# Lzcstan/DrugLAMP

Measured on AMD Instinct MI355X. Metric: drug-protein pairs/sec training step, higher is better.
Workload: dtype bf16; 1 GPU; DrugLAMP training step (cls step, epoch 1; fwd+bwd+grad all-reduce+AdamW), BindingDB-shaped synthetic pairs (512 drug nodes/tokens, 2304 protein tokens = 256 sites, pre-extracted 384-d/640-d LLM embeddings), global batch 256 = 256 per GPU x 1; per_gpu_batch=256, global_batch=256, parallelism=dp1, step_kind=cls, epoch=1, hip_graph=False, protein_seq_len=2304, distinct_batches=8, first_touch_steps=8, padding_rows=computed once, protein_cnn_rows=distinct rows, streams=independent branches on side HIP streams

## Files before the change

### druglamp_amd/_lib.py

```python
from __future__ import annotations

import ctypes as C
import os

import torch

_HERE = os.path.dirname(os.path.abspath(__file__))
_variant = os.environ.get("DL_USE_STUDY_LIB", "")
if _variant and not _variant.endswith(".so"):
    raise RuntimeError("DL_USE_STUDY_LIB=%s: the -DDL_STUDY build (libdruglamp_hip_study.so) was removed; commit 97fb613 is the last "
                       "that builds it (python -m druglamp_amd.build --study).  Only a variant library name (libdruglamp_hip_<variant>.so) "
                       "is accepted." % _variant)
LIB_PATH = os.path.join(_HERE, "lib", _variant or "libdruglamp_hip.so")

DL_F32, DL_BF16 = 0, 1

c_i64, c_i32, c_f32, c_u64, c_vp, c_sz = C.c_int64, C.c_int32, C.c_float, C.c_uint64, C.c_void_p, C.c_size_t


class ReduceItem(C.Structure):
    _fields_ = [
        ("kind", c_i32), ("out_dtype", c_i32),
        ("src", c_vp), ("out", c_vp),
        ("mn", c_i64), ("ldc", c_i64),
# ... 209 lines not shown
    "dl_pgca_pairs_ragged_profile": (c_i32, [C.POINTER(PgcaPairsRaggedProfileArgs), c_vp]),
    "dl_token_gate_fwd": (c_i32, [c_vp, c_vp, c_vp, c_vp, c_i64, c_i64, c_i64, c_i32, c_i32, c_i32, c_vp]),
    "dl_token_gate_bwd": (c_i32, [c_vp, c_vp, c_vp, c_vp, c_vp, c_i64, c_i64, c_i64, c_i32, c_i32, c_i32, c_vp]),
    "dl_gate_dpre": (c_i32, [c_vp, c_vp, c_vp, c_vp, c_i64, c_i64, c_i32, c_i32, c_vp]),
    "dl_add_rowmod_dropout": (c_i32, [c_vp, c_vp, c_vp, c_i64, c_i64, c_i64, c_f32, c_u64, c_vp, c_i32, c_vp]),
    "dl_dropout_apply": (c_i32, [c_vp, c_vp, c_i64, c_i64, c_i64, c_i64, c_f32, c_u64, c_vp, c_i32, c_vp]),
    "dl_fill_pool": (c_i32, [c_vp, c_vp, c_vp, c_i64, c_i64, c_i64, c_i32, c_i32, c_i32, c_vp]),
    "dl_cnn_sitepool_fwd": (c_i32, [c_vp, c_vp, c_i64, c_i64, c_i64, c_i32, c_i32, c_i32, c_vp]),
    "dl_cnn_sitepool_bwd": (c_i32, [c_vp, c_vp, c_i64, c_i64, c_i64, c_i32, c_i32, c_i32, c_vp]),
    "dl_bn_stats_finalize": (c_i32, [c_vp, c_i64, c_i64, c_i64, c_i64, c_i64, c_vp, c_i32, c_i64, c_f32, c_f32, c_vp, c_vp, c_vp, c_vp, c_vp, c_vp, c_vp, c_sz, c_vp]),
    "dl_bn_finalize": (c_i32, [c_vp, c_i64, c_f32, c_f32, c_vp, c_vp, c_vp, c_vp, c_vp, c_i64, c_vp]),
    "dl_interleave_streams": (c_i32, [c_vp, c_vp, c_i64, c_i64, c_i32, c_i32, c_vp]),
    "dl_norm_adjacency": (c_i32, [c_vp, c_vp, c_i64, c_i32, c_i32, c_vp]),
    "dl_graph_aggregate": (c_i32, [c_vp, c_vp, c_vp, c_i64, c_i32, c_i32, c_i32, c_i32, c_i32, c_vp]),
    "dl_concat2": (c_i32, [c_vp, c_vp, c_vp, c_i64, c_i64, c_i64, c_i32, c_vp]),
    "dl_gather_pad": (c_i32, [c_vp, c_vp, c_vp, c_vp, c_i64, c_i64, c_i64, c_i32, c_i32, c_vp]),
    "dl_embed_pad": (c_i32, [c_vp, c_vp, c_vp, c_vp, c_i64, c_i64, c_i32, c_i32, c_i32, c_i32, c_vp]),
    "dl_weight_prep": (c_i32, [c_vp, c_vp, c_i32, c_i32, c_vp]),
    "dl_gelu_bwd": (c_i32, [c_vp, c_vp, c_vp, c_i64, c_i32, c_vp]),
    "dl_cast": (c_i32, [c_vp, c_i32, c_vp, c_i32, c_i64, c_vp]),
    "dl_rowmod_sum": (c_i32, [c_vp, c_vp, c_i64, c_i64, c_i64, c_i32, c_i32, c_vp]),
    "dl_cos_rowloss_fwd": (c_i32, [c_vp, c_vp, c_vp, c_vp, c_i64, c_i64, c_vp]),
    "dl_cos_rowloss_bwd": (c_i32, [c_vp, c_vp, c_f32, c_vp, c_i64, c_i64, c_vp]),
    "dl_ntxent_fwd_ex": (c_i32, [C.POINTER(NtxentArgs), c_vp, c_vp, c_vp, c_vp]),
    "dl_ntxent_bwd_ex": (c_i32, [C.POINTER(NtxentArgs), c_f32, c_vp, c_vp, c_vp]),
    "dl_ntxent_workspace_bytes": (c_sz, [c_i64, c_i64]),
    "dl_ntxent_fwd": (c_i32, [c_vp, c_vp, c_i64, c_i64, c_f32, c_vp, c_vp, c_vp, c_sz, c_vp]),
    "dl_ntxent_bwd": (c_i32, [c_vp, c_vp, c_i64, c_i64, c_f32, c_vp, c_f32, c_vp, c_vp, c_vp]),
    "dl_triplet_sigcos_buffer_floats": (c_sz, [c_i64, c_i64]),
    "dl_triplet_sigcos_fwd": (c_i32, [c_vp, c_vp, c_vp, c_i64, c_i64, c_i64, c_f32, c_vp, c_vp, c_vp, c_vp]),
    "dl_triplet_sigcos_bwd": (c_i32, [c_vp, c_vp, c_vp, c_vp, c_i64, c_i64, c_i64, c_f32, c_vp, c_f32, c_vp, c_vp, c_vp]),
    "dl_adamw_step": (c_i32, [c_vp, c_vp, c_vp, c_vp, c_i64, c_f32, c_f32, c_f32, c_f32, c_f32, c_i64, c_f32, c_vp,
                              c_i32, c_vp]),
    "dl_bn_stats_rw": (c_i32, [c_vp, c_i64, c_i64, c_vp, c_i32, c_vp, c_vp, c_sz, c_vp]),
    "dl_bn_apply_fwd_rw": (c_i32, [c_vp, c_vp, c_vp, c_vp, c_vp, c_vp, c_i64, c_i64, c_vp, c_i32, c_vp]),
    "dl_bn_bwd_reduce_rw": (c_i32, [c_vp, c_vp, c_vp, c_vp, c_i64, c_i64, c_vp, c_i32, c_vp, c_vp, c_sz, c_vp]),
    "dl_bn_bwd_apply_rw": (c_i32, [c_vp, c_vp, c_vp, c_vp, c_vp, c_vp, c_f32, c_i32, c_vp, c_i64, c_i64, c_vp, c_i32, c_vp]),
    "dl_bn_eval_bwd": (c_i32, [c_vp, c_vp, c_vp, c_vp, c_vp, c_vp, c_i32, c_i32, c_vp, c_vp, c_i64, c_i64, c_i64, c_i64, c_i64, c_vp, c_i32,
                               c_vp, c_sz, c_vp]),
    "dl_cnn_sitepool_rows_fwd": (c_i32, [c_vp, c_vp, c_vp, c_i64, c_i64, c_i64, c_i32, c_i32, c_vp]),
    "dl_cnn_sitepool_rows_bwd": (c_i32, [c_vp, c_vp, c_vp, c_vp, c_i64, c_i64, c_i64, c_i64, c_i32, c_i32, c_vp]),
    "dl_embed_rows": (c_i32, [c_vp, c_vp, c_vp, c_vp, c_vp, c_i64, c_i32, c_i32, c_vp, c_i64, c_i64, c_vp, c_i32, c_vp]),
    "dl_rows_gather": (c_i32, [c_vp, c_vp, c_vp, c_i64, c_i64, c_vp]),
    "dl_rows_sum_strided": (c_i32, [c_vp, c_vp, c_vp, c_i64, c_i64, c_i32, c_vp]),
    "dl_rows_equal_check": (c_i32, [c_vp, c_i64, c_i64, c_i64, c_i64, C.c_uint32, c_vp, c_vp]),
    "dl_ce_rows_workspace_bytes": (c_sz, [c_i64]),
    "dl_ce_rows_fwd": (c_i32, [c_vp, c_i64, c_vp, c_i64, c_i32, c_i64, c_i32, c_vp, c_vp, c_vp, c_sz, c_vp]),
    "dl_ce_rows_bwd": (c_i32, [c_vp, c_i64, c_vp, c_i64, c_i32, c_i64, c_i32, c_vp, c_vp, c_vp, c_vp, c_i64, c_i32, c_vp]),
    "dl_protein_plan_build": (c_i32, [c_vp, c_i64, c_i64, c_i64, c_vp, c_vp, c_vp, c_vp, c_vp, c_vp, c_vp]),
    "dl_prof_enable": (c_i32, [c_i32, c_i32]),
    "dl_prof_collect": (c_i32, [c_i32, C.POINTER(c_i64), C.POINTER(C.c_double), C.POINTER(C.c_double),
                                C.POINTER(C.c_double)]),
    "dl_prof_totals": (c_i32, [c_i32, C.POINTER(c_i64), C.POINTER(C.c_double), C.POINTER(C.c_double)]),
    "dl_prof_collect_tag": (c_i32, [c_i32, c_i32, C.POINTER(c_i64), C.POINTER(C.c_double), C.POINTER(C.c_double), C.POINTER(C.c_double),
                                    C.POINTER(c_i64), C.POINTER(C.c_double), C.POINTER(C.c_double)]),
}

_lib = None

AUDIT = os.environ.get("DL_GRAPH_PTR_AUDIT") == "1"
_audit_log = None


def audit_begin() -> None:
    global _audit_log
    _audit_log = []
# ... 80 lines not shown
```

### druglamp_amd/build.py

```python
from __future__ import annotations

import os
import subprocess
import sys
from concurrent.futures import ThreadPoolExecutor

HERE = os.path.dirname(os.path.abspath(__file__))
CSRC = os.path.join(HERE, "csrc")
LIBDIR = os.path.join(HERE, "lib")
OBJDIR = os.path.join(LIBDIR, "obj")
LIB = os.path.join(LIBDIR, "libdruglamp_hip.so")
ARCH = "gfx950"
HIPCC = os.environ.get("HIPCC", "/opt/rocm/bin/hipcc")
FLAGS = ["--offload-arch=" + ARCH, "-O3", "-std=c++17", "-fPIC", "-Wno-unused-result"] + os.environ.get("DL_EXTRA_HIPCC_FLAGS", "").split()


def _sources():
    return sorted(f for f in os.listdir(CSRC) if f.endswith(".hip"))


def _headers():
    hs = [os.path.join(CSRC, f) for f in os.listdir(CSRC) if f.endswith(".cuh")]
    hs.append(os.path.join(os.path.dirname(HERE), "include", "druglamp_hip.h"))
    return hs


def csrc_hash() -> str:
    import hashlib
    h = hashlib.sha1()
    files = [os.path.join(CSRC, f) for f in sorted(os.listdir(CSRC)) if f.endswith((".hip", ".cuh"))]
    files.append(os.path.join(os.path.dirname(HERE), "include", "druglamp_hip.h"))
    for f in files:
        h.update(os.path.basename(f).encode() + b"\0")
        with open(f, "rb") as fh:
            h.update(fh.read())
    return h.hexdigest()


def _stale(out, deps):
    if not os.path.exists(out):
        return True
    t = os.path.getmtime(out)
    return any(os.path.getmtime(d) > t for d in deps)


FILE_FLAGS = {"norm.hip": ["-fno-slp-vectorize"], "elementwise.hip": ["-fno-slp-vectorize"], "bn_eval.hip": ["-fno-slp-vectorize"]}


def _compile(src, force, objdir=OBJDIR, extra=()):
    obj = os.path.join(objdir, src[:-4] + ".o")
    path = os.path.join(CSRC, src)
    if force or _stale(obj, [path] + _headers() + [os.path.abspath(__file__)]):
        keep = os.environ.get("DL_BUILD_NOSLP_FILES")
        ff = FILE_FLAGS.get(src, []) if (keep is None or src in keep.split(",")) else []
        if src in os.environ.get("DL_BUILD_NOSLP_EXTRA", "").split(","):
            ff = ff + ["-fno-slp-vectorize"]
        cmd = [HIPCC] + FLAGS + ff + list(extra) + ["-c", path, "-o", obj]
        r = subprocess.run(cmd, capture_output=True, text=True)
        if r.returncode != 0:
            raise RuntimeError("hipcc failed for %s:\n%s\n%s" % (src, r.stdout, r.stderr))
    return obj


def build(force: bool = False, verbose: bool = True, variant: str = "", defines=()) -> str:
    objdir = OBJDIR + ("_" + variant if variant else "")
    lib = LIB.replace(".so", "_%s.so" % variant) if variant else LIB
    extra = tuple(defines)
    os.makedirs(objdir, exist_ok=True)
    srcs = _sources()
    with ThreadPoolExecutor(max_workers=min(6, len(srcs))) as ex:
        objs = list(ex.map(lambda s: _compile(s, force, objdir, extra), srcs))
    return _link(lib, objs, force, verbose)


def _link(LIB, objs, force, verbose):
    if force or _stale(LIB, objs):
        cmd = [HIPCC, "--offload-arch=" + ARCH, "-shared", "-fPIC", "-o", LIB] + objs
        r = subprocess.run(cmd, capture_output=True, text=True)
        if r.returncode != 0:
# ... 18 lines not shown
```

### druglamp_amd/functional.py

```python
from __future__ import annotations

import functools
import contextlib
import os
import math
import weakref
from typing import List, Optional, Sequence

import torch

from . import ops

_param_epoch = 0
def _maybe_deferring():
    return contextlib.nullcontext() if os.environ.get("DL_DEFER_REDUCTIONS", "1") == "0" else ops.deferred_reductions()


def _deferring(fn):
    if os.environ.get("DL_DEFER_REDUCTIONS", "1") == "0":
        return fn

    @functools.wraps(fn)
    def wrapped(*a, **k):
        with ops.deferred_reductions():
# ... 1196 lines not shown
            ticks, _tick_list = _tick_list, None
            if ticks and exc[0] is None:
                cnt = {}
                for t in ticks:
                    e = cnt.setdefault(id(t), [t, 0])
                    e[1] += 1
                with torch.no_grad():
                    for k in sorted({c for _, c in cnt.values()}):
                        torch._foreach_add_([t for t, c in cnt.values() if c == k], k)
        return False


def bn_tick(counter: torch.Tensor) -> None:
    if _tick_list is not None:
        _tick_list.append(counter)
    else:
        with torch.no_grad():
            counter += 1


def batch_norm_rows(bn: torch.nn.BatchNorm1d, x2d: torch.Tensor, relu: bool = False) -> torch.Tensor:
    C = x2d.shape[1]
    if bn.training and x2d.shape[0] <= 1:
        raise ValueError("Expected more than 1 value per channel when training, got input size {}".format(x2d.size()))
    w = bn.weight if bn.weight is not None else torch.ones(C, device=x2d.device)
    b = bn.bias if bn.bias is not None else torch.zeros(C, device=x2d.device)
    y, mean, var = BatchNormRowsFn.apply(x2d, w, b, bn.running_mean, bn.running_var, bn.training, bn.eps,
                                         bn.momentum if bn.training else None, relu)
    if bn.training:
        bn_tick(bn.num_batches_tracked)
    return y


def run_mlp(seq, x: torch.Tensor, tail=None) -> torch.Tensor:
    import torch.nn as nn
    layers = list(seq)
    i = 0
    while i < len(layers):
        layer = layers[i]
        if isinstance(layer, nn.Linear):
            if x.shape[-1] < layer.in_features:
                raise ValueError("run_mlp: input narrower than the layer")
            x = dense(x, layer.weight, layer.bias)
        elif isinstance(layer, nn.BatchNorm1d):
            if x.shape[-1] != layer.num_features:
                x = x[:, :layer.num_features].contiguous()
            fuse = i + 1 < len(layers) and isinstance(layers[i + 1], nn.ReLU)
            if tail is not None and layer.training:
                x = batch_norm_rows_weighted_tail(layer, x, *tail, relu=fuse)
            else:
                x = batch_norm_rows(layer, x, relu=fuse)
            i += 1 if fuse else 0
        elif isinstance(layer, nn.ReLU):
            x = torch.relu(x)
        else:
            raise NotImplementedError("run_mlp: %s" % type(layer).__name__)
        i += 1
    return x
```

### druglamp_amd/model/basic_model.py

```python
from __future__ import annotations

import contextlib

import os

import torch
import torch.nn as nn
import torch.nn.functional as F

from .. import functional as Fn
from .. import ops
from .. import screening
from ..configs import get_model_defaults
from .cross_modality import CrossModality
from .PGCA import GuidedCrossAttention
from .PMMA import MultiHeadLinearAttention, PairedMultimodelAttention
from .self_supervised_learning import SSL

from .._lib import FLAG_DRUG_TOKEN_PAD as _FLAG_TOK, FLAG_GCN_NODE_PAD as _FLAG_GCN

_TAIL_ROWS = 8

CONFIGS = {"LAMP": get_model_defaults}

# ... 165 lines not shown
        if bn_training:
            for bn in (self.bn1, self.bn2, self.bn3):
                Fn.bn_tick(bn.num_batches_tracked)
        if fused_pool:
            return z
        z = z.transpose(1, 2).contiguous().view(B, L, C)
        if site_pool:
            z = z.view(B, int(site_pool), L // int(site_pool), C).mean(dim=1)
        return z


class FeedForwardLayer(nn.Module):
    def __init__(self, d_in, d_h):
        super().__init__()
        self.lin1 = nn.Linear(d_in, d_h)
        self.lin2 = nn.Linear(d_h, d_in)
        self.act = nn.GELU()
        self.norm = nn.LayerNorm(d_h)

    def forward(self, x):
        return self.lin2(self.norm(self.act(self.lin1(x))))


class MLP(nn.Module):
    def __init__(self, in_dim, hidden_dim, out_dim, binary=1):
        super().__init__()
        self.fc1 = nn.Linear(in_dim, hidden_dim)
        self.bn1 = nn.BatchNorm1d(hidden_dim)
        self.fc2 = nn.Linear(hidden_dim, hidden_dim)
        self.bn2 = nn.BatchNorm1d(hidden_dim)
        self.fc3 = nn.Linear(hidden_dim, out_dim)
        self.bn3 = nn.BatchNorm1d(out_dim)
        self.fc4 = nn.Linear(out_dim, binary)

    compute_dtype = torch.float32

    def forward(self, x):
        x = Fn.cast(x, self.compute_dtype)
        for fc, bn in ((self.fc1, self.bn1), (self.fc2, self.bn2), (self.fc3, self.bn3)):
            x = Fn.batch_norm_rows(bn, Fn.dense(x, fc.weight, fc.bias, act=True))
        return Fn.dense(x, self.fc4.weight, self.fc4.bias)[:, :self.fc4.out_features]


class DrugLAMPBase(nn.Module):
    llm_branch = True

    def __init__(self, n_drug_feature, n_prot_feature, n_hidden=128, **cfg):
        super().__init__()
        self.site_len = cfg["PROTEIN"]["SITE_LEN"]
        self.seq_len_q = cfg["PROTEIN"]["SEQ_LEN"]
        dec = cfg["DECODER"]
        self.compact_padding = os.environ.get("DL_PAD_COMPACT", "1") != "0"
        self.check_padding = os.environ.get("DL_PAD_CHECK", "0") == "1"
        self.guard_padding = os.environ.get("DL_PAD_GUARD", "1") != "0"
        self.compact_cnn = os.environ.get("DL_CNN_COMPACT", "1") != "0"
        self.compact_keys = os.environ.get("DL_KEY_COMPACT", "1") != "0"
        self.branch_streams = os.environ.get("DL_BRANCH_STREAMS", "1") != "0"
        self._streams = None
        self.drug_extractor = MolecularGCN(in_feats=cfg["DRUG"]["NODE_IN_FEATS"], dim_embedding=n_hidden,
                                           padding=cfg["DRUG"]["PADDING"], hidden_feats=[n_hidden] * 3)
        self.protein_extractor = ProteinCNN(n_hidden, [n_hidden] * 3, cfg["PROTEIN"]["KERNEL_SIZE"],
                                            cfg["PROTEIN"]["PADDING"])
        self.ssl_model = SSL(prot_extractor=self.protein_extractor, n_prot_feature=n_prot_feature,
                             drug_ssl_type=str(cfg["RS"].get("DRUG_SSL_TYPE", "simsiam")), n_hidden=n_hidden,
                             global_batch=bool(cfg["RS"].get("GLOBAL_BATCH", False)))
        self.cm_model = CrossModality(use_cm=True, hidden_size=n_hidden, max_margin=cfg["RS"]["MAX_MARGIN"],
                                      n_re=cfg["RS"]["RESET_EPOCH"], global_batch=bool(cfg["RS"].get("GLOBAL_BATCH", False)))
        if self.seq_len_q % self.site_len:
            raise ValueError("PROTEIN.SEQ_LEN (%d) must be a multiple of PROTEIN.SITE_LEN (%d)" % (self.seq_len_q, self.site_len))
        model_cfg = CONFIGS["LAMP"](n_hidden, feat_len=self.seq_len_q // self.site_len)

        self.lin_d1 = nn.Linear(n_drug_feature + 1, 2 * n_hidden)
# ... 297 lines not shown
```

### druglamp_amd/ops.py

```python
from __future__ import annotations

import contextlib
import ctypes as C
import math
import os
from typing import Optional

import torch

from . import _lib
from ._lib import (DL_BF16, DL_F32, AttnBwdArgs, AttnFwdArgs, AttnProbsArgs, GemmArgs, PgcaPairsArgs, PgcaPairsProbsArgs, PgcaPairsProfileArgs,
                   PgcaPairsRaggedArgs, PgcaPairsRaggedProbsArgs, PgcaPairsRaggedProfileArgs, check)

_DT = {torch.float32: DL_F32, torch.bfloat16: DL_BF16}


def _dt(t: torch.Tensor) -> int:
    try:
        return _DT[t.dtype]
    except KeyError:
        raise TypeError("druglamp_amd: unsupported dtype %s (float32 / bfloat16 only)" % t.dtype)


_raw_stream = getattr(torch._C, "_cuda_getCurrentRawStream", None)
# ... 871 lines not shown
    lse = torch.empty(N, dtype=torch.float32, device=logits2d.device)
    out2 = torch.empty(2, dtype=torch.float32, device=logits2d.device)
    ws = _ws2.get(L.dl_ce_rows_workspace_bytes(N), logits2d.device)
    check(L.dl_ce_rows_fwd(logits2d.data_ptr(), ld, labels.data_ptr(), N, C, int(ignore_index), _dt(logits2d), lse.data_ptr(),
                           out2.data_ptr(), ws.data_ptr(), ws.numel(), _stream()), "dl_ce_rows_fwd")
    return out2, lse


def ce_rows_bwd(logits2d, labels, C: int, ignore_index: int, lse, out2, grad_out):
    N, Cp = logits2d.shape
    d = torch.empty((N, Cp), dtype=logits2d.dtype, device=logits2d.device)
    check(_lib.lib().dl_ce_rows_bwd(logits2d.data_ptr(), logits2d.stride(0), labels.data_ptr(), N, C, int(ignore_index), _dt(logits2d),
                                    lse.data_ptr(), out2.data_ptr(), grad_out.data_ptr(), d.data_ptr(), Cp, Cp, _stream()), "dl_ce_rows_bwd")
    return d


def gate_dpre(dl2d, w2, pre2d):
    _need_gpu(dl2d, w2, pre2d)
    M, H = dl2d.shape
    dd = pre2d.shape[1]
    out = torch.empty_like(pre2d)
    check(_lib.lib().dl_gate_dpre(dl2d.data_ptr(), w2.data_ptr(), pre2d.data_ptr(), out.data_ptr(), M, dd, H, _dt(pre2d), _stream()),
          "dl_gate_dpre")
    return out


def gelu_bwd(dy2d, pre2d):
    dx = torch.empty_like(dy2d)
    check(_lib.lib().dl_gelu_bwd(dy2d.data_ptr(), pre2d.data_ptr(), dx.data_ptr(), dy2d.numel(), _dt(dy2d), _stream()),
          "dl_gelu_bwd")
    return dx


def fill_pool(x: torch.Tensor, site_len: int, out_dtype: torch.dtype):
    _need_gpu(x)
    x = x.contiguous()
    B, S, F = x.shape
    Fp = (F + 1 + 7) // 8 * 8
    fill = torch.empty((B, S), dtype=x.dtype, device=x.device)
    pooled = torch.empty((B, S // site_len, Fp), dtype=out_dtype, device=x.device)
    check(_lib.lib().dl_fill_pool(x.data_ptr(), fill.data_ptr(), pooled.data_ptr(), B, S, F, site_len, _dt(x),
                                  _DT[out_dtype], _stream()), "dl_fill_pool")
    return fill, pooled


_weight_prep_launches = 0


def weight_prep_launches() -> int:
    return _weight_prep_launches


def weight_prep(items_dev: torch.Tensor, block_map_dev: torch.Tensor, n_blocks: int, out_dtype: torch.dtype) -> None:
    global _weight_prep_launches
    _need_gpu(items_dev, block_map_dev)
    _weight_prep_launches += 1
    check(_lib.lib().dl_weight_prep(items_dev.data_ptr(), block_map_dev.data_ptr(), int(n_blocks), _DT[out_dtype],
                                    _stream()), "dl_weight_prep")


def cnn_sitepool_fwd(z: torch.Tensor, L: int, halo: int, site_len: int) -> torch.Tensor:
    _need_gpu(z)
    B, LP, C = z.shape
    out = torch.empty((B, L // site_len, C), dtype=z.dtype, device=z.device)
    check(_lib.lib().dl_cnn_sitepool_fwd(z.data_ptr(), out.data_ptr(), B, L, C, halo, site_len, _dt(z), _stream()),
          "dl_cnn_sitepool_fwd")
# ... 208 lines not shown
```

### include/druglamp_hip.h

```cpp
#ifndef DRUGLAMP_HIP_H
#define DRUGLAMP_HIP_H

#include <stddef.h>
#include <stdint.h>

#ifdef __cplusplus
extern "C" {
#endif

typedef enum { DL_OK = 0, DL_ERR_ARG = -1, DL_ERR_SHAPE = -2, DL_ERR_ALIGN = -3,
               DL_ERR_WORKSPACE = -4, DL_ERR_LAUNCH = -5, DL_ERR_UNSUPPORTED = -6 } dl_status;

typedef enum { DL_F32 = 0, DL_BF16 = 1 } dl_dtype;

typedef void* dl_stream;

const char* dl_last_error(void);
int dl_version(void);

typedef struct dl_reduce_item {
  int32_t kind;
  int32_t out_dtype;
  const float* src;
  void* out;
// ... 50 lines not shown
int dl_bn_stats(const void* y, int64_t R, int64_t C, int64_t win, int64_t halo, int64_t valid,
                int32_t dtype, float* sums, void* workspace, size_t workspace_bytes, dl_stream s);
int dl_bn_finalize(const float* sums, int64_t n, float eps, float momentum, float* mean, float* var, float* rstd,
                   float* running_mean, float* running_var, int64_t C, dl_stream s);
int dl_bn_apply_fwd(const void* y, void* z, const float* mean, const float* rstd, const float* gamma,
                    const float* beta, int64_t R, int64_t C, int64_t win, int64_t halo, int64_t valid,
                    int32_t dtype, dl_stream s);
int dl_bn_bwd_reduce(const void* dz, const void* y, const float* mean, const float* rstd, int64_t R,
                     int64_t C, int64_t win, int64_t halo, int64_t valid, int32_t dtype, float* sums,
                     void* workspace, size_t workspace_bytes, dl_stream s);
int dl_bn_bwd_apply(const void* dz, const void* y, const float* mean, const float* rstd,
                    const float* gamma, const float* sums, float inv_n, int32_t relu_mask, void* dy,
                    int64_t R, int64_t C, int64_t win, int64_t halo, int64_t valid, int32_t dtype,
                    dl_stream s);
int dl_bn_stats_rw(const void* y, int64_t R, int64_t C, const float* row_w, int32_t dtype, float* sums, void* workspace,
                   size_t workspace_bytes, dl_stream s);
int dl_bn_stats_finalize(const void* y, int64_t R, int64_t C, int64_t win, int64_t halo, int64_t valid, const float* row_w,
                         int32_t dtype, int64_t n, float eps, float momentum, float* sums, float* mean, float* var, float* rstd,
                         float* running_mean, float* running_var, void* workspace, size_t workspace_bytes, dl_stream s);
int dl_bn_apply_fwd_rw(const void* y, void* z, const float* mean, const float* rstd, const float* gamma, const float* beta,
                       int64_t R, int64_t C, const float* row_w, int32_t dtype, dl_stream s);
int dl_bn_bwd_reduce_rw(const void* dz, const void* y, const float* mean, const float* rstd, int64_t R, int64_t C,
                        const float* row_w, int32_t dtype, float* sums, void* workspace, size_t workspace_bytes, dl_stream s);
int dl_bn_bwd_apply_rw(const void* dz, const void* y, const float* mean, const float* rstd, const float* gamma,
                       const float* sums, float inv_n, int32_t relu_mask, void* dy, int64_t R, int64_t C, const float* row_w,
                       int32_t dtype, dl_stream s);
int dl_bn_tail_fix(void* dy, const void* y, const float* mean, const float* rstd, const float* gamma, const float* sums,
                   float inv_n, int32_t w, int64_t R, int64_t C, int64_t win, int64_t lead, int32_t dtype, dl_stream s);
int dl_bn_apply_relu_fwd(const void* y, void* z, const float* mean, const float* rstd, const float* gamma, const float* beta,
                         int64_t R, int64_t C, int32_t dtype, dl_stream s);
int dl_bn_relu_bwd(const void* dz, const void* y, const float* mean, const float* rstd, const float* gamma, const float* beta,
                   float inv_n, void* dy, float* sums, int64_t R, int64_t C, int32_t dtype, void* workspace, size_t workspace_bytes,
                   dl_stream s);
int dl_bn_eval_bwd(const void* dz, const void* y, const float* mean, const float* rstd, const float* gamma, const float* beta,
                   int32_t relu_in, int32_t relu_out, void* dy, float* sums, int64_t R, int64_t C, int64_t win, int64_t halo,
                   int64_t valid, const float* row_w, int32_t dtype, void* workspace, size_t workspace_bytes, dl_stream s);

int dl_layernorm_fwd(const void* x, int64_t ldx, const float* gamma, const float* beta, void* y,
                     int64_t ldy, float* mean, float* rstd, int64_t M, int64_t D, float eps,
                     int32_t dtype, dl_stream s);
size_t dl_layernorm_bwd_workspace_bytes(int64_t M, int64_t D);
int dl_layernorm_bwd(const void* dy, int64_t lddy, int64_t dy_share, const void* x, int64_t ldx, const float* mean,
                     const float* rstd, const float* gamma, const void* dres, int64_t lddres,
                     void* dx, int64_t lddx, float* dgamma, float* dbeta, int32_t accumulate,
                     int64_t M, int64_t D, int32_t dtype, void* workspace, size_t workspace_bytes,
                     dl_reduce_item* deferred, dl_stream s);

typedef struct {
  const void* Q; const void* K; const void* V; void* O; float* LSE; float* raw_logits;
  int64_t q_ps, q_hs, q_rs, k_ps, k_hs, k_rs, v_ps, v_hs, v_rs, o_ps, o_hs, o_rs, o_ss;
  int32_t n_problems, n_heads, n_segments, partner_shift, Lq, Lk, head_dim, dtype;
  float scale;
  int32_t algo;
  int32_t key_tail_rows;
  float key_tail_weight;
} dl_attn_fwd_args;
enum { DL_ATTN_ALGO_AUTO = 0, DL_ATTN_ALGO_STREAM = 1, DL_ATTN_ALGO_TWO_PASS = 2, DL_ATTN_ALGO_ONE_PASS = 3 };
int dl_attn_fwd(const dl_attn_fwd_args* a, dl_stream s);

typedef struct {
  const void* Q; const void* K; const void* V; const void* O; const void* dO;
  const float* LSE; float* Delta;
  void* dQ; void* dK; void* dV;
  int64_t q_ps, q_hs, q_rs, k_ps, k_hs, k_rs, v_ps, v_hs, v_rs, o_ps, o_hs, o_rs, o_ss;
  int64_t do_ps, do_hs, do_rs, do_ss, dq_ps, dq_hs, dq_rs, dk_ps, dk_hs, dk_rs, dv_ps, dv_hs, dv_rs;
  int32_t n_problems, n_heads, n_segments, partner_shift, Lq, Lk, head_dim, dtype;
// ... 209 lines not shown
```

Measured before the change: 21250 pairs/s.

## Fuse MLP head Linear+GELU+BatchNorm into single forward and backward kernels

Adds HIP kernels that run each decoder-head layer (linear, bias, GELU, training-mode BatchNorm with running-stat update) in one workgroup per 32 output columns, holding every batch row so the column statistics are reduced on chip. The backward kernel fuses the BN and GELU gradients with the dbias/dgamma/dbeta reductions and computes dW slices over a K-split grid; dx still uses a separate GEMM. The goal is to cut kernel launches and intermediate round trips through memory for these small MLP layers. It is enabled by default for bf16 batches of up to 256 rows and adds narrow shape constraints; grids are small (N/32 workgroups), so occupancy may be low.

Measured after the change: 21370 pairs/s, median of 4. Within noise of the previous version (+0.6%).

```diff
diff --git a/druglamp_amd/_lib.py b/druglamp_amd/_lib.py
--- a/druglamp_amd/_lib.py
+++ b/druglamp_amd/_lib.py
@@ -265,6 +265,8 @@
     "dl_triplet_sigcos_bwd": (c_i32, [c_vp, c_vp, c_vp, c_vp, c_i64, c_i64, c_i64, c_f32, c_vp, c_f32, c_vp, c_vp, c_vp]),
     "dl_adamw_step": (c_i32, [c_vp, c_vp, c_vp, c_vp, c_i64, c_f32, c_f32, c_f32, c_f32, c_f32, c_i64, c_f32, c_vp,
                               c_i32, c_vp]),
+    "dl_head_layer_fwd": (c_i32, [c_vp, c_vp, c_vp, c_vp, c_vp, c_vp, c_vp, c_vp, c_vp, c_vp, c_vp, c_i64, c_i64, c_i64, c_f32, c_f32, c_i32, c_vp]),
+    "dl_head_layer_bwd": (c_i32, [c_vp, c_vp, c_vp, c_vp, c_vp, c_vp, c_vp, c_vp, c_vp, c_vp, c_vp, c_i64, c_i64, c_i64, c_i32, c_vp]),
     "dl_bn_stats_rw": (c_i32, [c_vp, c_i64, c_i64, c_vp, c_i32, c_vp, c_vp, c_sz, c_vp]),
     "dl_bn_apply_fwd_rw": (c_i32, [c_vp, c_vp, c_vp, c_vp, c_vp, c_vp, c_i64, c_i64, c_vp, c_i32, c_vp]),
     "dl_bn_bwd_reduce_rw": (c_i32, [c_vp, c_vp, c_vp, c_vp, c_i64, c_i64, c_vp, c_i32, c_vp, c_vp, c_sz, c_vp]),
diff --git a/druglamp_amd/build.py b/druglamp_amd/build.py
--- a/druglamp_amd/build.py
+++ b/druglamp_amd/build.py
@@ -44,7 +44,8 @@
     return any(os.path.getmtime(d) > t for d in deps)
 
 
-FILE_FLAGS = {"norm.hip": ["-fno-slp-vectorize"], "elementwise.hip": ["-fno-slp-vectorize"], "bn_eval.hip": ["-fno-slp-vectorize"]}
+FILE_FLAGS = {"norm.hip": ["-fno-slp-vectorize"], "elementwise.hip": ["-fno-slp-vectorize"], "bn_eval.hip": ["-fno-slp-vectorize"],
+              "head.hip": ["-fno-slp-vectorize"]}
 
 
 def _compile(src, force, objdir=OBJDIR, extra=()):
diff --git a/druglamp_amd/csrc/head.hip b/druglamp_amd/csrc/head.hip
--- /dev/null
+++ b/druglamp_amd/csrc/head.hip
@@ -0,0 +1,350 @@
+#include "tiles.cuh"
+
+namespace {
+using namespace dltile;
+
+constexpr int HL_ROWS = 256;
+constexpr int HL_COLS = 32;
+constexpr int HL_KC = 64;
+constexpr int HL_KSPAN = 128;
+constexpr int HL_PF = 4;
+using XT = ATile<bf16_t, HL_KC>;
+
+template <int NR> struct ChunkStager {
+  static_assert((NR * XT::CPR) % 256 == 0, "every thread stages the same number of 16-byte pieces");
+  static constexpr int NCH = NR * XT::CPR / 256;
+  u32x4 r[NCH];
+  uint32_t ok;
+  __device__ __forceinline__ void load(const bf16_t* __restrict__ base, int64_t ld, int row0, int row_limit, int col0, int col_limit) {
+    ok = 0u;
+#pragma unroll
+    for (int i = 0; i < NCH; ++i) {
+      const int c = threadIdx.x + i * 256;
+      const int row = row0 + c / XT::CPR, col = col0 + (c % XT::CPR) * 8;
+      if (row < row_limit && col < col_limit) ok |= 1u << i;
+      r[i] = *reinterpret_cast<const u32x4*>(base + (int64_t)min(row, row_limit - 1) * ld + min(col, col_limit - 8));
+    }
+  }
+  __device__ __forceinline__ void store(char* lds) const {
+#pragma unroll
+    for (int i = 0; i < NCH; ++i) {
+      const int c = threadIdx.x + i * 256;
+      const int row = c / XT::CPR, ch = c % XT::CPR;
+      lds_write16(lds, row * XT::RB + ((ch ^ XT::swz(row)) << 4), ((ok >> i) & 1u) ? r[i] : u32x4{0u, 0u, 0u, 0u});
+    }
+  }
+};
+
+__device__ __forceinline__ f32x4 unpack4(u32x2 w) { return f32x4{bf16lo(w[0]), bf16hi(w[0]), bf16lo(w[1]), bf16hi(w[1])}; }
+__device__ __forceinline__ u32x2 pack4(f32x4 v) { return u32x2{pack_bf16x2(v[0], v[1]), pack_bf16x2(v[2], v[3])}; }
+
+template <int ROUNDS>
+__global__ __launch_bounds__(256) void head_layer_fwd_kernel(const bf16_t* __restrict__ x, const bf16_t* __restrict__ w,
+                                                             const float* __restrict__ bias, const float* __restrict__ gamma,
+                                                             const float* __restrict__ beta, bf16_t* __restrict__ z, bf16_t* __restrict__ y,
+                                                             float* __restrict__ mean, float* __restrict__ rstd, float* __restrict__ rmean,
+                                                             float* __restrict__ rvar, int M, int N, int K, float eps, float momentum,
+                                                             float unbias) {
+  __shared__ __attribute__((aligned(16))) char Xs[HL_ROWS * XT::RB];
+  __shared__ __attribute__((aligned(16))) char Ws[HL_COLS * XT::RB];
+  __shared__ float red[4][HL_COLS];
+  __shared__ __attribute__((aligned(16))) float col_mean[HL_COLS];
+  __shared__ __attribute__((aligned(16))) float col_rstd[HL_COLS];
+  const int tid = threadIdx.x, lane = tid & 63, wave = tid >> 6, il = lane & 15, g = lane >> 4;
+  const int n0 = blockIdx.x * HL_COLS;
+  const int wrow = wave * 64;
+  int nrt = (M - wrow + 15) / 16;
+  nrt = nrt < 0 ? 0 : (nrt > 4 ? 4 : nrt);
+
+  f32x4 acc[2][4];
+#pragma unroll
+  for (int ct = 0; ct < 2; ++ct)
+#pragma unroll
+    for (int rt = 0; rt < 4; ++rt) acc[ct][rt] = f32x4{0.f, 0.f, 0.f, 0.f};
+
+  ChunkStager<HL_ROWS> sx[HL_PF];
+  ChunkStager<HL_COLS> sw[HL_PF];
+#pragma unroll
+  for (int s = 0; s < HL_PF; ++s) {
+    sx[s].load(x, K, 0, M, s * HL_KC, K);
+    sw[s].load(w, K, n0, N, s * HL_KC, K);
+  }
+#pragma unroll
+  for (int r = 0; r < ROUNDS; ++r) {
+#pragma unroll
+    for (int s = 0; s < HL_PF; ++s) {
+      const int k0 = (r * HL_PF + s) * HL_KC;
+      __syncthreads();
+      sx[s].store(Xs);
+      sw[s].store(Ws);
+      __syncthreads();
+      if (r + 1 < ROUNDS) {
+        sx[s].load(x, K, 0, M, k0 + HL_PF * HL_KC, K);
+        sw[s].load(w, K, n0, N, k0 + HL_PF * HL_KC, K);
+      }
+      if (k0 < K) {
+#pragma unroll
+        for (int kf = 0; kf < HL_KC / 32; ++kf) {
+          const u32x4 wa0 = frag_kc<bf16_t, HL_KC>(Ws, 0, kf, il, g), wa1 = frag_kc<bf16_t, HL_KC>(Ws, 16, kf, il, g);
+#pragma unroll
+          for (int rt = 0; rt < 4; ++rt) {
+            if (rt < nrt) {
+              const u32x4 xb = frag_kc<bf16_t, HL_KC>(Xs, wrow + rt * 16, kf, il, g);
+              acc[0][rt] = Mma<bf16_t>::mma(wa0, xb, acc[0][rt]);
+              acc[1][rt] = Mma<bf16_t>::mma(wa1, xb, acc[1][rt]);
+            }
+          }
+        }
+      }
+    }
+  }
+
+  int col[2];
+  bool colok[2];
+  f32x4 b4[2];
+#pragma unroll
+  for (int ct = 0; ct < 2; ++ct) {
+    col[ct] = n0 + ct * 16 + 4 * g;
+    colok[ct] = col[ct] < N;
+    b4[ct] = colok[ct] ? *reinterpret_cast<const f32x4*>(bias + col[ct]) : f32x4{0.f, 0.f, 0.f, 0.f};
+  }
+  f32x4 s[2] = {f32x4{0.f, 0.f, 0.f, 0.f}, f32x4{0.f, 0.f, 0.f, 0.f}};
+#pragma unroll
+  for (int ct = 0; ct < 2; ++ct)
+#pragma unroll
+    for (int rt = 0; rt < 4; ++rt) {
+      const int row = wrow + rt * 16 + il;
+      const bool ok = row < M;
+      const u32x2 zb = pack4(acc[ct][rt] + b4[ct]);
+      if (ok && colok[ct]) *reinterpret_cast<u32x2*>(z + (int64_t)row * N + col[ct]) = zb;
+      const f32x4 a = gelu4<bf16_t>(unpack4(zb));
+      acc[ct][rt] = a;
+      if (ok) s[ct] += a;
+    }
+#pragma unroll
+  for (int ct = 0; ct < 2; ++ct)
+#pragma unroll
+    for (int r = 0; r < 4; ++r) {
+      const float t = row16_sum(s[ct][r]);
+      if (il == 0) red[wave][ct * 16 + 4 * g + r] = t;
+    }
+  __syncthreads();
+  const float inv_m = 1.f / (float)M;
+  if (tid < HL_COLS) col_mean[tid] = (((red[0][tid] + red[1][tid]) + red[2][tid]) + red[3][tid]) * inv_m;
+  __syncthreads();
+  f32x4 mu[2];
+#pragma unroll
+  for (int ct = 0; ct < 2; ++ct) {
+    mu[ct] = *reinterpret_cast<const f32x4*>(&col_mean[ct * 16 + 4 * g]);
+    s[ct] = f32x4{0.f, 0.f, 0.f, 0.f};
+#pragma unroll
+    for (int rt = 0; rt < 4; ++rt) {
+      const f32x4 d = acc[ct][rt] - mu[ct];
+      acc[ct][rt] = d;
+      if (wrow + rt * 16 + il < M) s[ct] += d * d;
+    }
+  }
+#pragma unroll
+  for (int ct = 0; ct < 2; ++ct)
+#pragma unroll
+    for (int r = 0; r < 4; ++r) {
+      const float t = row16_sum(s[ct][r]);
+      if (il == 0) red[wave][ct * 16 + 4 * g + r] = t;
+    }
+  __syncthreads();
+  if (tid < HL_COLS) {
+    const float var = (((red[0][tid] + red[1][tid]) + red[2][tid]) + red[3][tid]) * inv_m;
+    const float rs = rsqrtf(var + eps);
+    col_rstd[tid] = rs;
+    const int c = n0 + tid;
+    if (c < N) {
+      const float m = col_mean[tid];
+      mean[c] = m;
+      rstd[c] = rs;
+      if (rmean) rmean[c] = (1.f - momentum) * rmean[c] + momentum * m;
+      if (rvar) rvar[c] = (1.f - momentum) * rvar[c] + momentum * (var * unbias);
+    }
+  }
+  __syncthreads();
+#pragma unroll
+  for (int ct = 0; ct < 2; ++ct) {
+    if (!colok[ct]) continue;
+    const f32x4 rs = *reinterpret_cast<const f32x4*>(&col_rstd[ct * 16 + 4 * g]);
+    const f32x4 ga = *reinterpret_cast<const f32x4*>(gamma + col[ct]), be = *reinterpret_cast<const f32x4*>(beta + col[ct]);
+#pragma unroll
+    for (int rt = 0; rt < 4; ++rt) {
+      const int row = wrow + rt * 16 + il;
+      if (row < M) *reinterpret_cast<u32x2*>(y + (int64_t)row * N + col[ct]) = pack4(acc[ct][rt] * rs * ga + be);
+    }
+  }
+}
+
+struct DzTile {
+  static constexpr int RB = HL_COLS * 2;
+  __device__ static __forceinline__ int off(int row, int col) {
+    const int b = col * 2;
+    return row * RB + ((((b >> 4) ^ ((row >> 2) & 3))) << 4) + (b & 15);
+  }
+};
+__device__ __forceinline__ u32x4 dz_frag_tr(const char* lds, int rbase, int colbase, int il, int g) {
+  const int r0 = rbase + 4 * g + (il >> 2);
+  const int col = colbase + (il & 3) * 4;
+  const u32x2 a = lds_read_tr16(lds, DzTile::off(r0, col));
+  const u32x2 b = lds_read_tr16(lds, DzTile::off(r0 + 16, col));
+  return u32x4{a[0], a[1], b[0], b[1]};
+}
+
+__device__ __forceinline__ void colsum32(float (*red)[HL_COLS], float* out) {
+  __syncthreads();
+  if (threadIdx.x < HL_COLS) {
+    float t = 0.f;
+#pragma unroll
+    for (int k = 0; k < 32; ++k) t += red[k][threadIdx.x];
+    out[threadIdx.x] = t;
+  }
+  __syncthreads();
+}
+
+__global__ __launch_bounds__(256) void head_layer_bwd_kernel(const bf16_t* __restrict__ dy, const bf16_t* __restrict__ z,
+                                                             const float* __restrict__ mean, const float* __restrict__ rstd,
+                                                             const float* __restrict__ gamma, const bf16_t* __restrict__ xin,
+                                                             bf16_t* __restrict__ dz, float* __restrict__ dW, float* __restrict__ dbias,
+                                                             float* __restrict__ dgamma, float* __restrict__ dbeta, int M, int N, int K) {
+  __shared__ __attribute__((aligned(16))) char Xs[HL_ROWS * XT::RB];
+  __shared__ __attribute__((aligned(16))) char Ds[HL_ROWS * DzTile::RB];
+  __shared__ float red[32][HL_COLS];
+  __shared__ __attribute__((aligned(16))) float sum0[HL_COLS];
+  __shared__ __attribute__((aligned(16))) float sum1[HL_COLS];
+  const int tid = threadIdx.x, lane = tid & 63, wave = tid >> 6, il = lane & 15, g = lane >> 4;
+  const int n0 = blockIdx.x * HL_COLS;
+  const int kbeg = blockIdx.y * HL_KSPAN;
+  const int kend = min(K, kbeg + HL_KSPAN);
+  const bool first = blockIdx.y == 0;
+
+  static_assert(HL_KSPAN == 2 * HL_KC, "the two stagers below hold the workgroup's whole x_in span");
+  ChunkStager<HL_ROWS> sx[2];
+  sx[0].load(xin, K, 0, M, kbeg, K);
+  sx[1].load(xin, K, 0, M, kbeg + HL_KC, K);
+
+  const int cl = (tid & 7) * 4, rsub = tid >> 3;
+  const int cq = n0 + cl;
+  const bool colok = cq < N;
+  f32x4 mu = {0.f, 0.f, 0.f, 0.f}, rs = mu, ga = mu;
+  if (colok) {
+    mu = *reinterpret_cast<const f32x4*>(mean + cq);
+    rs = *reinterpret_cast<const f32x4*>(rstd + cq);
+    ga = *reinterpret_cast<const f32x4*>(gamma + cq);
+  }
+  f32x4 d[8], zr[8], xh[8];
+  f32x4 s0 = {0.f, 0.f, 0.f, 0.f}, s1 = s0;
+#pragma unroll
+  for (int j = 0; j < 8; ++j) {
+    const int row = rsub + 32 * j;
+    d[j] = f32x4{0.f, 0.f, 0.f, 0.f};
+    zr[j] = d[j];
+    if (colok && row < M) {
+      d[j] = unpack4(*reinterpret_cast<const u32x2*>(dy + (int64_t)row * N + cq));
+      zr[j] = unpack4(*reinterpret_cast<const u32x2*>(z + (int64_t)row * N + cq));
+    }
+    xh[j] = (gelu4<bf16_t>(zr[j]) - mu) * rs;
+    if (row < M) { s0 += d[j]; s1 += d[j] * xh[j]; }
+  }
+#pragma unroll
+  for (int e = 0; e < 4; ++e) red[rsub][cl + e] = s0[e];
+  colsum32(red, sum0);
+#pragma unroll
+  for (int e = 0; e < 4; ++e) red[rsub][cl + e] = s1[e];
+  colsum32(red, sum1);
+  const float inv_m = 1.f / (float)M;
+  const f32x4 m0 = *reinterpret_cast<const f32x4*>(&sum0[cl]) * inv_m, m1 = *reinterpret_cast<const f32x4*>(&sum1[cl]) * inv_m;
+  const f32x4 gr = ga * rs;
+  f32x4 s2 = {0.f, 0.f, 0.f, 0.f};
+#pragma unroll
+  for (int j = 0; j < 8; ++j) {
+    const int row = rsub + 32 * j;
+    f32x4 v = {0.f, 0.f, 0.f, 0.f};
+    if (colok && row < M) {
+      const f32x4 da = gr * (d[j] - m0 - xh[j] * m1);
+      v = da * gelu_grad4<bf16_t>(zr[j]);
+      s2 += v;
+    }
+    const u32x2 vb = pack4(v);
+    *reinterpret_cast<u32x2*>(Ds + DzTile::off(row, cl)) = vb;
+    if (first && colok && row < M) *reinterpret_cast<u32x2*>(dz + (int64_t)row * N + cq) = vb;
+  }
+  if (first && tid < HL_COLS && n0 + tid < N) { dbeta[n0 + tid] = sum0[tid]; dgamma[n0 + tid] = sum1[tid]; }
+#pragma unroll
+  for (int e = 0; e < 4; ++e) red[rsub][cl + e] = s2[e];
+  colsum32(red, sum0);
+  if (first && tid < HL_COLS && n0 + tid < N) dbias[n0 + tid] = sum0[tid];
+
+  const int nfr = (M + 31) / 32;
+#pragma unroll
+  for (int s = 0; s < 2; ++s) {
+    const int k0 = kbeg + s * HL_KC;
+    if (k0 >= kend) break;
+    __syncthreads();
+    sx[s].store(Xs);
+    __syncthreads();
+    f32x4 acc[2] = {f32x4{0.f, 0.f, 0.f, 0.f}, f32x4{0.f, 0.f, 0.f, 0.f}};
+    for (int f = 0; f < nfr; ++f) {
+      const u32x4 xa = frag_tr<bf16_t, HL_KC>(Xs, f * 32, wave * 16, il, g);
+      acc[0] = Mma<bf16_t>::mma(xa, dz_frag_tr(Ds, f * 32, 0, il, g), acc[0]);
+      acc[1] = Mma<bf16_t>::mma(xa, dz_frag_tr(Ds, f * 32, 16, il, g), acc[1]);
+    }
+    const int kc = k0 + wave * 16 + 4 * g;
+    if (kc < K) {
+#pragma unroll
+      for (int nt = 0; nt < 2; ++nt) {
+        const int n = n0 + nt * 16 + il;
+        if (n < N) *reinterpret_cast<f32x4*>(dW + (int64_t)n * K + kc) = acc[nt];
+      }
+    }
+  }
+}
+
+static int head_check(const char* who, int64_t M, int64_t N, int64_t K, int32_t dtype) {
+  DL_CHECK_ARG(dtype == DL_BF16, DL_ERR_UNSUPPORTED, "%s: bf16 only", who);
+  DL_CHECK_ARG(M >= 2 && M <= HL_ROWS, DL_ERR_SHAPE, "%s: M = %lld rows, 2 .. %d are supported (a workgroup owns every row of its columns)", who,
+               (long long)M, HL_ROWS);
+  DL_CHECK_ARG(N >= 8 && N <= 1024 && N % 8 == 0 && K >= 8 && K <= 1024 && K % 8 == 0, DL_ERR_SHAPE,
+               "%s: N = %lld, K = %lld must be multiples of 8 in 8 .. 1024", who, (long long)N, (long long)K);
+  return DL_OK;
+}
+}
+
+extern "C" int dl_head_layer_fwd(const void* x, const void* w, const float* bias, const float* gamma, const float* beta, void* z, void* y,
+                                 float* mean, float* rstd, float* running_mean, float* running_var, int64_t M, int64_t N, int64_t K,
+                                 float eps, float momentum, int32_t dtype, dl_stream stream) {
+  DL_CHECK_ARG(x && w && bias && gamma && beta && z && y && mean && rstd, DL_ERR_ARG, "dl_head_layer_fwd: null pointer");
+  DL_CHECK_ARG((running_mean == nullptr) == (running_var == nullptr), DL_ERR_ARG, "dl_head_layer_fwd: running_mean and running_var go together");
+  const int rc = head_check("dl_head_layer_fwd", M, N, K, dtype);
+  if (rc != DL_OK) return rc;
+  DL_CHECK_ARG(eps > 0.f, DL_ERR_ARG, "dl_head_layer_fwd: eps must be positive");
+  DL_CHECK_ARG((((uintptr_t)x | (uintptr_t)w | (uintptr_t)z | (uintptr_t)y | (uintptr_t)bias | (uintptr_t)gamma | (uintptr_t)beta) & 15) == 0, DL_ERR_ALIGN,
+               "dl_head_layer_fwd: x, w, z, y, bias, gamma and beta must be 16-byte aligned");
+  const float unbias = (float)((double)M / (double)(M - 1));
+#define HEAD_FWD(R) hipLaunchKernelGGL((head_layer_fwd_kernel<R>), dim3((uint32_t)((N + HL_COLS - 1) / HL_COLS)), dim3(256), 0, (hipStream_t)stream, \
+                                       (const bf16_t*)x, (const bf16_t*)w, bias, gamma, beta, (bf16_t*)z, (bf16_t*)y, mean, rstd, running_mean,       \
+                                       running_var, (int)M, (int)N, (int)K, eps, momentum, unbias)
+  const int rounds = (int)((K + HL_PF * HL_KC - 1) / (HL_PF * HL_KC));
+  if (rounds == 1) HEAD_FWD(1); else if (rounds == 2) HEAD_FWD(2); else if (rounds == 3) HEAD_FWD(3); else HEAD_FWD(4);
+#undef HEAD_FWD
+  DL_CHECK_LAUNCH("dl_head_layer_fwd");
+  return DL_OK;
+}
+
+extern "C" int dl_head_layer_bwd(const void* dy, const void* z, const float* mean, const float* rstd, const float* gamma, const void* x_in,
+                                 void* dz, float* dW, float* dbias, float* dgamma, float* dbeta, int64_t M, int64_t N, int64_t K,
+                                 int32_t dtype, dl_stream stream) {
+  DL_CHECK_ARG(dy && z && mean && rstd && gamma && x_in && dz && dW && dbias && dgamma && dbeta, DL_ERR_ARG, "dl_head_layer_bwd: null pointer");
+  const int rc = head_check("dl_head_layer_bwd", M, N, K, dtype);
+  if (rc != DL_OK) return rc;
+  DL_CHECK_ARG((((uintptr_t)dy | (uintptr_t)z | (uintptr_t)x_in | (uintptr_t)dz | (uintptr_t)dW | (uintptr_t)mean | (uintptr_t)rstd | (uintptr_t)gamma) & 15) == 0,
+               DL_ERR_ALIGN, "dl_head_layer_bwd: dy, z, x_in, dz, dW, mean, rstd and gamma must be 16-byte aligned");
+  hipLaunchKernelGGL(head_layer_bwd_kernel, dim3((uint32_t)((N + HL_COLS - 1) / HL_COLS), (uint32_t)((K + HL_KSPAN - 1) / HL_KSPAN)), dim3(256), 0,
+                     (hipStream_t)stream, (const bf16_t*)dy, (const bf16_t*)z, mean, rstd, gamma, (const bf16_t*)x_in, (bf16_t*)dz, dW, dbias,
+                     dgamma, dbeta, (int)M, (int)N, (int)K);
+  DL_CHECK_LAUNCH("dl_head_layer_bwd");
+  return DL_OK;
+}
diff --git a/druglamp_amd/functional.py b/druglamp_amd/functional.py
--- a/druglamp_amd/functional.py
+++ b/druglamp_amd/functional.py
@@ -1252,6 +1252,48 @@
     return y
 
 
+class HeadLayerFn(torch.autograd.Function):
+
+    @staticmethod
+    def forward(ctx, x, weight, bias, gamma, beta, rmean, rvar, eps, momentum):
+        x2 = x.contiguous()
+        cdt = x2.dtype
+        N, K = weight.shape
+        w = _padded_weight(weight, N, K, cdt)
+        wT = lowp((weight,), cdt, transpose=True, pad=(N, K)) if ctx.needs_input_grad[0] else None
+        g = gamma.detach()
+        y, z, mean, rstd = ops.head_layer_fwd(x2, w, bias.detach(), g, beta.detach(), eps, momentum, rmean, rvar)
+        ctx.save_for_backward(x2, z, mean, rstd, g, wT)
+        return y
+
+    @staticmethod
+    def backward(ctx, dy):
+        x2, z, mean, rstd, g, wT = ctx.saved_tensors
+        M, K = x2.shape
+        N = z.shape[1]
+        dz, dW, db, dg, dbeta = ops.head_layer_bwd(dy.contiguous(), z, mean, rstd, g, x2)
+        dx = ops.gemm(dz, wT, M=M, N=K, K=N) if wT is not None else None
+        return dx, dW, db, dg, dbeta, None, None, None, None
+
+
+def head_layer_fusable(fc: torch.nn.Linear, bn: torch.nn.BatchNorm1d, x2d: torch.Tensor) -> bool:
+    if not (x2d.is_cuda and x2d.dim() == 2 and x2d.dtype == torch.bfloat16 and bn.training):
+        return False
+    if not (isinstance(bn.momentum, float) and bn.weight is not None and bn.bias is not None and fc.bias is not None and
+            bn.running_mean is not None and bn.running_var is not None):
+        return False
+    if any(t.dtype != torch.float32 for t in (fc.weight, fc.bias, bn.weight, bn.bias, bn.running_mean, bn.running_var)):
+        return False
+    N, K = fc.weight.shape
+    return x2d.shape[1] == K and bn.num_features == N and ops.head_layer_supported(x2d.shape[0], N, K, x2d.dtype)
+
+
+def head_layer(fc: torch.nn.Linear, bn: torch.nn.BatchNorm1d, x2d: torch.Tensor) -> torch.Tensor:
+    y = HeadLayerFn.apply(x2d, fc.weight, fc.bias, bn.weight, bn.bias, bn.running_mean, bn.running_var, bn.eps, bn.momentum)
+    bn_tick(bn.num_batches_tracked)
+    return y
+
+
 def run_mlp(seq, x: torch.Tensor, tail=None) -> torch.Tensor:
     import torch.nn as nn
     layers = list(seq)
diff --git a/druglamp_amd/model/basic_model.py b/druglamp_amd/model/basic_model.py
--- a/druglamp_amd/model/basic_model.py
+++ b/druglamp_amd/model/basic_model.py
@@ -221,12 +221,16 @@
         self.fc3 = nn.Linear(hidden_dim, out_dim)
         self.bn3 = nn.BatchNorm1d(out_dim)
         self.fc4 = nn.Linear(out_dim, binary)
+        self.head_fused = os.environ.get("DL_HEAD_FUSED", "1") != "0"
 
     compute_dtype = torch.float32
 
     def forward(self, x):
         x = Fn.cast(x, self.compute_dtype)
         for fc, bn in ((self.fc1, self.bn1), (self.fc2, self.bn2), (self.fc3, self.bn3)):
+            if self.head_fused and x.dim() == 2 and Fn.head_layer_fusable(fc, bn, x):
+                x = Fn.head_layer(fc, bn, x)
+                continue
             x = Fn.batch_norm_rows(bn, Fn.dense(x, fc.weight, fc.bias, act=True))
         return Fn.dense(x, self.fc4.weight, self.fc4.bias)[:, :self.fc4.out_features]
 
diff --git a/druglamp_amd/ops.py b/druglamp_amd/ops.py
--- a/druglamp_amd/ops.py
+++ b/druglamp_amd/ops.py
@@ -927,6 +927,36 @@
     return dx
 
 
+def head_layer_supported(M: int, N: int, K: int, dtype) -> bool:
+    return dtype == torch.bfloat16 and 2 <= M <= 256 and 8 <= N <= 1024 and 8 <= K <= 1024 and N % 8 == 0 and K % 8 == 0
+
+
+def head_layer_fwd(x2d, w, bias, gamma, beta, eps, momentum=0.0, running_mean=None, running_var=None):
+    _need_gpu(x2d, w, bias, gamma, beta)
+    M, K = x2d.shape
+    N = w.shape[0]
+    z = torch.empty((M, N), dtype=x2d.dtype, device=x2d.device)
+    y = torch.empty_like(z)
+    stats = torch.empty((2, N), dtype=torch.float32, device=x2d.device)
+    check(_lib.lib().dl_head_layer_fwd(x2d.data_ptr(), w.data_ptr(), bias.data_ptr(), gamma.data_ptr(), beta.data_ptr(), z.data_ptr(), y.data_ptr(),
+                                       stats[0].data_ptr(), stats[1].data_ptr(), _ptr(running_mean), _ptr(running_var), M, N, K, float(eps),
+                                       float(momentum), _dt(x2d), _stream()), "dl_head_layer_fwd")
+    return y, z, stats[0], stats[1]
+
+
+def head_layer_bwd(dy2d, z, mean, rstd, gamma, x_in):
+    _need_gpu(dy2d, z, x_in)
+    M, N = z.shape
+    K = x_in.shape[1]
+    dz = torch.empty_like(z)
+    dW = torch.empty((N, K), dtype=torch.float32, device=z.device)
+    dv = torch.empty((3, N), dtype=torch.float32, device=z.device)
+    check(_lib.lib().dl_head_layer_bwd(dy2d.data_ptr(), z.data_ptr(), mean.data_ptr(), rstd.data_ptr(), gamma.data_ptr(), x_in.data_ptr(),
+                                       dz.data_ptr(), dW.data_ptr(), dv[0].data_ptr(), dv[1].data_ptr(), dv[2].data_ptr(), M, N, K, _dt(z),
+                                       _stream()), "dl_head_layer_bwd")
+    return dz, dW, dv[0], dv[1], dv[2]
+
+
 def fill_pool(x: torch.Tensor, site_len: int, out_dtype: torch.dtype):
     _need_gpu(x)
     x = x.contiguous()
diff --git a/include/druglamp_hip.h b/include/druglamp_hip.h
--- a/include/druglamp_hip.h
+++ b/include/druglamp_hip.h
@@ -106,6 +106,12 @@
 int dl_bn_relu_bwd(const void* dz, const void* y, const float* mean, const float* rstd, const float* gamma, const float* beta,
                    float inv_n, void* dy, float* sums, int64_t R, int64_t C, int32_t dtype, void* workspace, size_t workspace_bytes,
                    dl_stream s);
+int dl_head_layer_fwd(const void* x, const void* w, const float* bias, const float* gamma, const float* beta, void* z, void* y,
+                      float* mean, float* rstd, float* running_mean, float* running_var, int64_t M, int64_t N, int64_t K,
+                      float eps, float momentum, int32_t dtype, dl_stream s);
+int dl_head_layer_bwd(const void* dy, const void* z, const float* mean, const float* rstd, const float* gamma, const void* x_in,
+                      void* dz, float* dW, float* dbias, float* dgamma, float* dbeta, int64_t M, int64_t N, int64_t K,
+                      int32_t dtype, dl_stream s);
 int dl_bn_eval_bwd(const void* dz, const void* y, const float* mean, const float* rstd, const float* gamma, const float* beta,
                    int32_t relu_in, int32_t relu_out, void* dy, float* sums, int64_t R, int64_t C, int64_t win, int64_t halo,
                    int64_t valid, const float* row_w, int32_t dtype, void* workspace, size_t workspace_bytes, dl_stream s);
```
